# IDSIA/hhmarl_2D

Hardware: AMD Instinct MI355X
Metric: env-steps/sec (2v2) (higher is better)
Workload: dtype f64

## Files before the change

### hhmarl_2d_amd/csrc/hh_device.h

```cpp
#ifndef HH_DEVICE_H
#define HH_DEVICE_H

#include <hip/hip_runtime.h>
#include <stdint.h>

#include "hh_abi.h"
#include "hh_envelope.h"
#include "hh_geodesic.h"
#include "hh_math.h"
#include "hh_rng.h"
#include "hh_spec.h"

#ifdef HH_NO_RARE
#define HH_RARE(x) (x)
#define HH_USUAL(x) (x)
#else
#define HH_RARE(x) __builtin_expect(!!(x), 0)
#define HH_USUAL(x) __builtin_expect(!!(x), 1)
#endif

#ifndef HH_BLOCK
#define HH_BLOCK 64
#endif

// ... 204 lines not shown
    P.cmd_hdg[u] = m.cmd_hdg; P.cmd_spd[u] = m.cmd_spd;
    int4 p;
    p.x = (m.cannon_remain & 0xffff) | ((m.cannon_max & 0xffff) << 16);
    p.y = (m.burst & 0xff) | ((m.missile_remain & 0xff) << 8) | ((m.rocket_max & 0xff) << 16) | ((m.missile_wait & 0xff) << 24);
    p.z = (m.ac_type & 0xff) | ((m.alive & 0xff) << 8) | ((m.has_missile & 0xff) << 16) | ((m.n_tgt & 0xff) << 24);
    p.w = (m.tgt0 & 0xff) | ((m.tgt1 & 0xff) << 8) | ((m.tgt2 & 0xff) << 16) | ((m.cmd_act & 0xff) << 24);
    P.pack[u] = p;
    P.tgt_d[u] = m.tgt_d0; P.tgt_d[U + u] = m.tgt_d1; P.tgt_d[2 * U + u] = m.tgt_d2;
    int2 r;
    r.x = (m.rk_alive & 0xff) | ((m.rk_target & 0xff) << 8) | ((m.rk_life & 0xff) << 16);
    if constexpr (X) {
        const UnitW &x = static_cast<const UnitW &>(m);
        r.x |= (int)(((unsigned)(x.tgt3 & 15) << 24) | ((unsigned)(x.tgt4 & 15) << 28));
        P.tgt_d[3 * U + u] = x.tgt_d3; P.tgt_d[4 * U + u] = x.tgt_d4;
    }
    r.y = m.rk_seq;
    P.rk_pack[u] = r;
    P.rk_lat[u] = m.rk_lat; P.rk_lon[u] = m.rk_lon; P.rk_hdg[u] = m.rk_hdg; P.rk_cmd[u] = m.rk_cmd;
}

__device__ __forceinline__ void arena_load(const DevPtrs &P, const DevCfg &c, int n, Arena &a) {
    int4 p = P.ar_pack[n];
    a.steps = p.x; a.episode = p.y;
    a.escaping = p.z & 0xff; a.escaping_time = (int)(int8_t)((p.z >> 8) & 0xff); a.done = (p.z >> 16) & 0xff;
    a.hl_s = (p.z >> 24) & 0x1f; a.hl_run = (p.z >> 29) & 1;
    a.next_seq = p.w;
    a.akey = hh_rng_arena_key(c.seed, c.arena_offset + (uint64_t)n);
    arena_rekey(a);
}

__device__ __forceinline__ void arena_store(const DevPtrs &P, int n, const Arena &a) {
    int4 p;
    p.x = a.steps; p.y = a.episode;
    p.z = (a.escaping & 0xff) | ((a.escaping_time & 0xff) << 8) | ((a.done & 0xff) << 16) | ((a.hl_s & 0x1f) << 24) | ((a.hl_run & 1) << 29);
    p.w = a.next_seq;
    P.ar_pack[n] = p;
}

__device__ __forceinline__ double d_normalize_angle(double a) {
    while (a >= 360.0) a -= 360.0;
    while (a < 0.0) a += 360.0;
    return a;
}
__device__ __forceinline__ double d_signed_heading_diff(double actual, double desired) {
    double delta = desired - actual;
    if (delta < -180.0) delta = 360.0 + delta;
    if (delta > 180.0) delta = -360.0 + delta;
    return delta;
}

__device__ __forceinline__ void d_dist_bearing(double lat1, double lon1, double lat2, double lon2, double &km, double &brg) {
    double s12, azi1;
    hh_geo_inverse(lat1, lon1, lat2, lon2, &s12, &azi1);
    km = s12 / 1000.0;
    brg = d_normalize_angle(azi1);
}

__device__ __forceinline__ int d_envelope_exact_body(int kind, int ac_type, double la1, double lo1, double la2, double lo2, double hdg) {
    double km, brg;
    d_dist_bearing(la1, lo1, la2, lo2, km, brg);
    if (kind == 0) {
        if (km <= HH_MISSILE_RANGE_KM) {
            double delta = hh_fabs(d_signed_heading_diff(d_normalize_angle(hdg + HH_MISSILE_HALF_DEG), brg));
            return (int)delta <= (int)HH_MISSILE_HALF_DEG;
        }
        return 0;
    }
    if (kind == 1) {
        if (km < HH_AC_CANNON_KM(ac_type)) return hh_fabs(d_signed_heading_diff(hdg, brg)) <= HH_AC_CANNON_HALF(ac_type);
        return 0;
    }
    return km < HH_ROCKET_FUSE_KM;
}
__device__ __noinline__ int d_envelope_exact(int kind, int ac_type, double la1, double lo1, double la2, double lo2, double hdg) {
    return d_envelope_exact_body(kind, ac_type, la1, lo1, la2, lo2, hdg);
}

__device__ __forceinline__ bool d_maybe_within_km(double lat1, double lon1, double lat2, double lon2, double r_km) {
    double lim = r_km / 100.0;
    bool near = hh_fabs(lat2 - lat1) <= lim && hh_fabs(lon2 - lon1) <= lim;
    bool lowlat = hh_fabs(lat1) < 25.0 && hh_fabs(lat2) < 25.0;
    return near || !lowlat;
}

__device__ __noinline__ void d_geo_direct_general(double lat1, double lon1, double azi1, double s12, double *lat2, double *lon2) {
    hh_geo_direct(lat1, lon1, azi1, s12, lat2, lon2);
}
__device__ __forceinline__ void d_geo_move(double lat1, double lon1, double azi1, double s12, double &lat2, double &lon2) {
    double a, b;
    if (HH_USUAL(s12 <= HH_GEO_SHORT_MAX_M && hh_fabs(lat1) <= HH_GEO_SHORT_MAX_LAT && hh_fabs(lon1) < 170.0 && hh_fabs(azi1) <= 360.0))
        hh_geo_direct_short(lat1, lon1, azi1, s12, &a, &b);
    else
        d_geo_direct_general(lat1, lon1, azi1, s12, &a, &b);
    lat2 = a;
    lon2 = b;
}

__device__ __forceinline__ void d_geo_move2(double lat_a, double lon_a, double azi_a, double s_a, double &lat2_a, double &lon2_a,
                                            double lat_b, double lon_b, double azi_b, double s_b, double &lat2_b, double &lon2_b) {
    bool ok_a = s_a <= HH_GEO_SHORT_MAX_M && hh_fabs(lat_a) <= HH_GEO_SHORT_MAX_LAT && hh_fabs(lon_a) < 170.0 && hh_fabs(azi_a) <= 360.0;
    bool ok_b = s_b <= HH_GEO_SHORT_MAX_M && hh_fabs(lat_b) <= HH_GEO_SHORT_MAX_LAT && hh_fabs(lon_b) < 170.0 && hh_fabs(azi_b) <= 360.0;
    if (HH_USUAL(ok_a && ok_b)) {
        double a0, a1, b0, b1;
        hh_geo_direct_short(lat_a, lon_a, azi_a, s_a, &a0, &a1);
        hh_geo_direct_short(lat_b, lon_b, azi_b, s_b, &b0, &b1);
        lat2_a = a0; lon2_a = a1; lat2_b = b0; lon2_b = b1;
    } else {
        d_geo_move(lat_a, lon_a, azi_a, s_a, lat2_a, lon2_a);
        d_geo_move(lat_b, lon_b, azi_b, s_b, lat2_b, lon2_b);
    }
}

__device__ __forceinline__ double d_rng(const Arena &a, int unit_id, int site, int sub) {
    return hh_rng_u01(a.tkey, (uint32_t)unit_id, (uint32_t)site, (uint32_t)sub);
}

#endif
```

### hhmarl_2d_amd/csrc/hh_kernels.h

```cpp
#ifndef HH_KERNELS_H
#define HH_KERNELS_H

#include "hh_device.h"

#ifdef HH_PROFILE_PHASES
__device__ unsigned long long hh_prof_cycles[24];
#define HH_PROF_DECL unsigned long long prof_t0_ = __builtin_readcyclecounter(), prof_acc_[14] = {0}
#define HH_PROF(k) do { unsigned long long t_ = __builtin_readcyclecounter(); prof_acc_[k] += t_ - prof_t0_; prof_t0_ = t_; } while (0)
#define HH_PROF_ARGS , unsigned long long &prof_t0_, unsigned long long *prof_acc_
#define HH_PROF_PASS , prof_t0_, prof_acc_
#define HH_PROF_FLUSH do { if ((threadIdx.x & 63) == 0) { for (int k_ = 0; k_ < 12; k_++) atomicAdd(&hh_prof_cycles[k_], prof_acc_[k_]); \
                                                          atomicAdd(&hh_prof_cycles[20], prof_acc_[12]); atomicAdd(&hh_prof_cycles[21], prof_acc_[13]); } } while (0)
#else
#define HH_PROF_DECL
#define HH_PROF(k)
#define HH_PROF_ARGS
#define HH_PROF_PASS
#define HH_PROF_FLUSH
#endif

template <int A, int B>
struct Shared {
    static constexpr int GPB = B / A;
    double lat0[B], lon0[B], hdg[B];
// ... 236 lines not shown
    if (mode != 2) out[n++] = (sh.flags[o] & FL_SHOT) ? 1.0f : 0.0f;
    return n;
}

template <int A, int B>
__device__ __forceinline__ void friend_block(const DevCfg &c, const Shared<A, B> &sh, int tid, int base, int s, int fj, float *out) {
    const int f = base + fj;
    if (sh_alive(sh, f)) {
        out[0] = sh.nlat[f];
        out[1] = sh.nlon[f];
        out[2] = (float)norm180(sh.p_foc[fj][tid]);
        out[3] = (float)norm180(sh.p_foc[s][f]);
        out[4] = (float)(c.inv_diag * sh.p_dist[fj][tid]);
    } else {
        out[0] = out[1] = out[2] = out[3] = out[4] = 0.0f;
    }
}

template <int A, int B>
__device__ __forceinline__ void lowlevel_obs(const DevCfg &c, const Shared<A, B> &sh, int tid, int base, int s, int mode, Unit &m, float *out, int D) {
    for (int k = 0; k < D; k++) out[k] = 0.0f;
    m.n_tgt = 0; m.tgt0 = 0; m.tgt_d0 = 0.0;
    if (!m.alive) return;
    Near3 nb;
    nearby(c, sh, tid, base, s, false, nb);
    if (nb.n == 0) return;
    m.n_tgt = 1; m.tgt0 = nb.i0 + 1; m.tgt_d0 = nb.d0;
    int fri = s < c.nA ? (s == 1 ? 0 : 1) : (s == 3 ? 2 : 3);
    int n = 0;
    out[n++] = sh.nlat[tid];
    out[n++] = sh.nlon[tid];
    out[n++] = sh.nspd[tid];
    out[n++] = sh.nhdg[tid];
    if (mode == HH_MODE_FIGHT) {
        const int oj = nb.i0;
        out[n++] = (float)norm180(sh.p_foc[oj][tid]);
        out[n++] = (float)aspect(sh.p_foc[s][base + oj]);
        out[n++] = sh.p_hd[oj][tid];
        out[n++] = (float)nb.d0;
        out[n++] = (float)hh_clip((double)m.cannon_remain / (double)m.cannon_max, 0.0, 1.0);
        if (m.ac_type == 1) {
            out[n++] = (float)hh_clip((double)m.missile_remain / (double)m.rocket_max, 0.0, 1.0);
            out[n++] = m.missile_wait == 0 ? 1.0f : 0.0f;
            out[n++] = (m.has_missile || m.burst > 0) ? 1.0f : 0.0f;
        } else {
            out[n++] = m.burst > 0 ? 1.0f : 0.0f;
        }
        n += opp_block(c, sh, 0, tid, base, s, oj, nb.d0, out + n);
    } else {
        out[n++] = (float)hh_clip((double)m.cannon_remain / (double)m.cannon_max, 0.0, 1.0);
        if (m.ac_type == 1) out[n++] = (float)hh_clip((double)m.missile_remain / (double)m.rocket_max, 0.0, 1.0);
        out[n++] = (sh.flags[tid] & FL_SHOT) ? 1.0f : 0.0f;
        opp_block(c, sh, 1, tid, base, s, nb.i0, nb.d0, out + n);
        if (nb.n >= 2) opp_block(c, sh, 1, tid, base, s, nb.i1, nb.d1, out + n + 9);
        n += 18;
    }
    friend_block(c, sh, tid, base, s, fri, out + n);
}

struct StepOut {
    double reward;
    int valid;
    int kill_event;
    double opp_stat0;
};

template <int GS, int B, bool INLINE_EXACT, class SH>
__device__ __forceinline__ void drain_envelope_queue_t(SH &sh, int tid, int count, int opp_id0) {
#ifdef HH_ABL_NO_ENVELOPE
    count = 0;
#endif
#pragma unroll 1
    for (int q = tid; q < count; q += B) {
        int code = sh.u.t.q_code[q];
        int src = code & 0xff, kind = (code >> 8) & 3, j = (code >> 10) & (GS > 8 ? 15 : 7);
        int ss = src % GS, sb = src - ss;
        double la1, lo1, la2, lo2;
        if (kind <= 1) { la1 = sh.lat0[src]; lo1 = sh.lon0[src]; }
        else { la1 = sh.u.t.rk_lat[src]; lo1 = sh.u.t.rk_lon[src]; }
        bool moved = kind >= 2 || (kind == 1 && j < ss);
        la2 = moved ? sh.u.t.lat1[sb + j] : sh.lat0[sb + j];
        lo2 = moved ? sh.u.t.lon1[sb + j] : sh.lon0[sb + j];
        const int t = (sh.flags[src] >> 1) & 3;
        const double hdg_src = kind == 0 ? sh.hdg[src] : sh.u.t.hdg1[src];
        const double sep = hh_max(hh_fabs(la2 - la1), hh_fabs(lo2 - lo1));
        const bool dom = hh_fabs(la1) <= HH_GEO_EST_MAX_LAT && hh_fabs(la2) <= HH_GEO_EST_MAX_LAT &&
                         hh_fabs(lo1) < 170.0 && hh_fabs(lo2) < 170.0;
        int verdict = -1;
        if (dom && sep <= (kind == 0 ? HH_GEO_EST_LONG_DEG : HH_GEO_EST_SHORT_DEG)) {
            double s_m, az;
            hh_geo_inverse_estimate(la1, lo1, la2, lo2, &s_m, &az);
            if (kind == 0) {
                double delta = hh_fabs(d_signed_heading_diff(d_normalize_angle(hdg_src + HH_MISSILE_HALF_DEG), az));
                if (s_m >= HH_MISSILE_RANGE_KM * 1000.0 + HH_GEO_EST_LONG_ABS_M) verdict = 0;
                else if (s_m <= HH_MISSILE_RANGE_KM * 1000.0 - HH_GEO_EST_LONG_ABS_M && s_m > HH_GEO_EST_MIN_M &&
                         hh_fabs(delta - (HH_MISSILE_HALF_DEG + 1.0)) > HH_GEO_EST_LONG_AZI)
                    verdict = delta < HH_MISSILE_HALF_DEG + 1.0;
            } else {
                const double r_m = (kind == 1 ? HH_AC_CANNON_KM(t) : HH_ROCKET_FUSE_KM) * 1000.0;
                const double eps = HH_GEO_EST_SHORT_REL * s_m + HH_GEO_EST_SHORT_ABS_M;
                if (s_m >= r_m + eps) verdict = 0;
                else if (s_m < r_m - eps && s_m > HH_GEO_EST_MIN_M) {
                    if (kind >= 2) verdict = 1;
                    else {
                        double d = hh_fabs(d_signed_heading_diff(hdg_src, az));
                        if (d <= HH_AC_CANNON_HALF(t) - HH_GEO_EST_SHORT_AZI) verdict = 1;
                        else if (d > HH_AC_CANNON_HALF(t) + HH_GEO_EST_SHORT_AZI) verdict = 0;
                    }
                }
            }
        }
#ifndef HH_ABL_NO_EXACT
        if (HH_RARE(verdict < 0)) verdict = INLINE_EXACT ? d_envelope_exact_body(kind, t, la1, lo1, la2, lo2, hdg_src)
                                                : d_envelope_exact(kind, t, la1, lo1, la2, lo2, hdg_src);
#endif
        int bit = 0;
        if (verdict) {
            if (kind == 0) bit = 1;
            else if (kind == 1) {
                const int id_src = GS == 8 ? (ss < 4 ? ss + 1 : opp_id0 + (ss - 4)) : ss + 1;
                const int id_tgt = GS == 8 ? (j < 4 ? j + 1 : opp_id0 + (j - 4)) : j + 1;
                double u = hh_rng_u01(sh.g_tkey[src / GS], (uint32_t)id_src, HH_SITE_CANNON, (uint32_t)id_tgt);
                if (u < HH_AC_HIT_PROB(t)) bit = 2 << j;
            } else bit = kind == 2 ? (1 << HH_RES_FUSE_BIT(GS)) : (1 << (HH_RES_FUSE_BIT(GS) + 1));
        }
        if (bit) atomicOr(&sh.res[src], bit);
    }
}
template <int A, int B, bool INLINE_EXACT = false>
__device__ __forceinline__ void drain_envelope_queue(Shared<A, B> &sh, int tid, int count) {
    drain_envelope_queue_t<A, B, INLINE_EXACT>(sh, tid, count, 0);
}

__device__ __forceinline__ void arm_cannon(Unit &m) {
    int b = HH_AC_BURST(m.ac_type);
    m.burst = m.cannon_remain < b ? m.cannon_remain : b;
}

template <int A, int B>
__device__ __forceinline__ int launch_planar(const Shared<A, B> &sh, int tid, int base, int j) {
    const double la = sh.lat0[tid], lo = sh.lon0[tid], tl = sh.lat0[base + j], to = sh.lon0[base + j];
    const double cross = sh.uc[tid] * (tl - la) - sh.us[tid] * (to - lo);
    return hh_missile_cone_planar(la, lo, tl, to, sh.p_foc[j][tid], cross, sh.p_dist[j][tid]);
}

template <int A, int B>
__device__ __forceinline__ int launch_planar_direct(const Shared<A, B> &sh, int tid, int base, int j) {
    const double la = sh.lat0[tid], lo = sh.lon0[tid], tl = sh.lat0[base + j], to = sh.lon0[base + j];
    const double c1 = sh.uc[tid], s1 = sh.us[tid], n1 = sh.un[tid];
    const double dx = to - lo, dy = tl - la;
    const double n2 = hh_sqrt(dx * dx + dy * dy);
    const double x = hh_clip((c1 * dx + s1 * dy) / (n1 * n2 + 1e-10), -1.0, 1.0);
    return hh_missile_cone_planar(la, lo, tl, to, hh_acos(x) * (180.0 / HH_PI), c1 * dy - s1 * dx, n2);
}

template <int A, int B, bool IX = false>
__device__ __forceinline__ void tick(const DevCfg &c, Shared<A, B> &sh, int tid, int g, int s, int base, bool active,
                                     Unit &m, Arena &ar, const int8_t *act, StepOut &out, uint32_t &ev_mask_out,
                                     const int tmode, const bool run_arena HH_PROF_ARGS) {
    const int id = s + 1;
    const bool running = tmode == 0 ? (active && !ar.done) : (active && run_arena);
    const bool agent = s < c.nA;
    const bool hl = c.env_kind == HH_ENV_HIGHLEVEL;
    if (tmode == 0) { out.reward = 0.0; out.valid = 0; }
    uint32_t evm = 0;
    out.kill_event = 0;
    if (running && tmode == 0) { ar.steps += 1; arena_rekey(ar); }
    const bool snap = running && m.alive;
    double opp_stat0 = tmode == 0 ? 0.0 : out.opp_stat0;
    int want_launch = 0, launch_tgt = 0;
    int wait_after = -1;
    bool base_gate = false;

    if (snap && tmode == 0) {
        if (agent || c.ext_opp) {
            int t = m.n_tgt ? m.tgt0 : 0;
            if (!agent) {
                Near3 nb;
                nearby(c, sh, tid, base, s, false, nb);
                m.n_tgt = nb.n ? 1 : 0; m.tgt0 = nb.n ? nb.i0 + 1 : 0; m.tgt_d0 = nb.n ? nb.d0 : 0.0;
                t = m.tgt0;
            } else {
                out.valid = 1;
                if (t && sh_alive(sh, base + t - 1)) opp_stat0 = norm180(sh.p_foc[s][base + t - 1]);
            }
            double nh = hh_pymod360(m.hdg + (double)(((int)act[0] - 6) * 15));
            if (nh >= 360.0 || nh < 0.0) nh = 0.0;
            m.cmd_hdg = nh;
            double mx = HH_AC_MAX_SPEED(m.ac_type);
            m.cmd_spd = 100.0 + ((mx - 100.0) / 8.0) * (double)act[1];
            bool agent_ll = agent && !hl;
            if (act[2] && m.cannon_remain > 0) {
                arm_cannon(m);
                if (agent_ll && c.agent_mode == HH_MODE_ESCAPE && m.cannon_remain < 90) out.reward -= 0.1;
            }
            if (m.ac_type == 1 && act[3]) {
                if (t && m.missile_remain > 0 && !m.has_missile && m.missile_wait == 0) {
                    base_gate = true;
                    want_launch = 1;
                    launch_tgt = t - 1;
                }
            }
        } else if (c.level <= 2) {
            if (c.level == 2) {
                arm_cannon(m);
                bool man = ar.steps <= 5;
                if (!man) man = (ar.steps % hh_rng_randint(d_rng(ar, id, HH_SITE_L2_PERIOD, 0), 35, 45)) <= 5;
// ... 739 lines not shown
```

### hhmarl_2d_amd/csrc/hh_kernels_oct.h

```cpp
#ifndef HH_KERNELS_OCT_H
#define HH_KERNELS_OCT_H

#include "hh_kernels_hier.h"

#define HH_DPP_QP(a, b, c, d) ((a) | ((b) << 2) | ((c) << 4) | ((d) << 6))
#define HH_DPP_ROW_SHL(n) (0x100 + (n))
#define HH_DPP_ROW_SHR(n) (0x110 + (n))

template <int CTRL>
__device__ __forceinline__ int o_perm_i(int v) { return __builtin_amdgcn_mov_dpp(v, CTRL, 0xf, 0xf, true); }
__device__ __forceinline__ int o_swap_i(int v) {
    const int a = __builtin_amdgcn_update_dpp(v, v, HH_DPP_ROW_SHL(4), 0xf, 0x5, false);
    return __builtin_amdgcn_update_dpp(a, v, HH_DPP_ROW_SHR(4), 0xf, 0xa, false);
}
template <int K>
__device__ __forceinline__ int o_rot_i(int v) {
    static_assert(K == 1 || K == 2, "ring of three");
    return o_perm_i<(K == 1 ? HH_DPP_QP(1, 2, 0, 3) : HH_DPP_QP(2, 0, 1, 3))>(v);
}
template <int P>
__device__ __forceinline__ int o_bc_i(int v) {
    const int t = o_perm_i<HH_DPP_QP(P & 3, P & 3, P & 3, P & 3)>(v);
    if (P < 4) return __builtin_amdgcn_update_dpp(t, t, HH_DPP_ROW_SHR(4), 0xf, 0xa, false);
    return __builtin_amdgcn_update_dpp(t, t, HH_DPP_ROW_SHL(4), 0xf, 0x5, false);
// ... 388 lines not shown
    out.kill_event = 0;
    const bool snap = running && L.exists && m.alive;
    const int amask0 = tb.amask;
    const int rk_age0 = (m.rk_alive && m.rk_life <= HH_ROCKET_MAX_LIFE) ? m.rk_life : 0;
    const double rk_speed0 = sh.rk_speed[rk_age0];

    const double lat_old = m.lat, lon_old = m.lon, hdg_old = m.hdg;
    bool fired = false;
    const int rk_pre = m.rk_alive;
    if (HH_USUAL(snap)) {
        const int t = m.ac_type;
        {
            const double delta = d_signed_heading_diff(m.hdg, m.cmd_hdg);
            const double max_deg = HH_AC_TURN_RATE(t) * 1.0;
            const double stepped = hh_pymod360(m.hdg + (delta >= 0.0 ? max_deg : -max_deg));
            const double nh = hh_fabs(delta) <= max_deg ? m.cmd_hdg : stepped;
            m.hdg = m.hdg != m.cmd_hdg ? nh : m.hdg;
        }
        {
            const double delta = m.cmd_spd - m.spd;
            const double max_delta = HH_AC_ACCEL(t) * 1.0;
            const double stepped = m.spd + (delta >= 0.0 ? max_delta : -max_delta);
            const double ns = hh_fabs(delta) <= max_delta ? m.cmd_spd : stepped;
            m.spd = m.spd != m.cmd_spd ? ns : m.spd;
        }
        {
            const bool f = m.burst > 0;
            const int b1 = m.burst - 1 > 0 ? m.burst - 1 : 0, c1 = m.cannon_remain - 1 > 0 ? m.cannon_remain - 1 : 0;
            fired = f;
            m.burst = f ? b1 : m.burst;
            m.cannon_remain = f ? c1 : m.cannon_remain;
        }
    }
    {
        const bool steer = snap & (m.has_missile != 0) & (m.rk_alive != 0);
        if (HH_USUAL(steer)) m.rk_cmd = hh_clip(m.rk_hdg * hh_rng_uniform(d_rng(ar, id, HH_SITE_ROCKET_NOISE, 0), 0.95, 1.05), 0.0, 359.0);
        m.has_missile = (snap & (m.has_missile != 0) & (m.rk_alive == 0)) ? 0 : m.has_missile;
    }
    const bool rk_spec = running && L.exists && rk_pre && m.rk_life <= HH_ROCKET_MAX_LIFE;
    double rk_nlat = 0.0, rk_nlon = 0.0, rk_nhdg = 0.0;
    {
        const bool mv_a = snap && m.spd > 0.0;
        const bool any_rk = __ballot(rk_spec) != 0ULL;
        if (HH_USUAL(any_rk)) {
            double r_hdg = m.rk_hdg;
            const double r_cmd = m.rk_cmd;
            {
                const double delta = d_signed_heading_diff(r_hdg, r_cmd);
                const double stepped = r_hdg + (delta >= 0.0 ? HH_ROCKET_TURN_RATE : -HH_ROCKET_TURN_RATE);
                const double nh = hh_fabs(delta) <= HH_ROCKET_TURN_RATE ? r_cmd : stepped;
                r_hdg = r_hdg != r_cmd ? nh : r_hdg;
            }
            rk_nhdg = r_hdg;
            double a_lat, a_lon;
            d_geo_move2(m.lat, m.lon, m.hdg, mv_a ? m.spd * HH_KNOTS_TO_MS * 1.0 : 0.0, a_lat, a_lon,
                        rk_spec ? m.rk_lat : 5.0, rk_spec ? m.rk_lon : 7.0, r_hdg, rk_speed0 * HH_KNOTS_TO_MS * 1.0, rk_nlat, rk_nlon);
            if (mv_a) { m.lat = a_lat; m.lon = a_lon; }
        } else {
            if (mv_a) d_geo_move(m.lat, m.lon, m.hdg, m.spd * HH_KNOTS_TO_MS * 1.0, m.lat, m.lon);
        }
    }
    const double rk0_lat = rk_pre ? m.rk_lat : lat_old, rk0_lon = rk_pre ? m.rk_lon : lon_old;
    OPub pn = pub;
    oct_publish_vec(m, pn);
    if (FULL) oct_publish_norm(c, m, pn);
    double lat1[5], lon1[5];
    HH_O_FETCH5(d, lat1, m.lat);
    HH_O_FETCH5(d, lon1, m.lon);

    const bool rk_maybe = running && L.exists && rk_pre;
    int q_total = 0;
    {
        const int t = m.ac_type;
        int push[5], pjs[5], any_push = 0;
#pragma unroll
        for (int r = 0; r < 5; r++) {
            const int pj = o_rel_pos(L, r);
            const bool snap_j = running && ((amask0 >> pj) & 1);
            const bool enemy = r >= 2;
            const bool lower = pj < L.p;
            const double tl = lower ? lat1[r] : tb.lat[r];
            const double to = lower ? lon1[r] : tb.lon[r];
            push[r] = (int)fired & (int)snap_j & ((int)(c.friendly_kill != 0) | (int)enemy) & (int)d_maybe_within_km(lat_old, lon_old, tl, to, HH_AC_CANNON_KM(t)) &
                      (int)!hh_cannon_cone_planar_outside(lat_old, lon_old, tl, to, pn.uc, pn.us, t);
            pjs[r] = pj;
            any_push |= push[r];
        }
        if (HH_RARE(o_any(any_push != 0))) {
#pragma unroll
            for (int r = 0; r < 5; r++) HH_O_PUSH(push[r] != 0, tid | (1 << 8) | (pjs[r] << 10));
        }
        if (o_any(rk_maybe)) {
            const int tp = rk_maybe ? o_slot_pos(c, m.rk_target - 1) : ((1 - L.q) << 2);
            const int rt = o_pos_rel(L, tp);
            HH_O_PUSH(rk_maybe && d_maybe_within_km(rk0_lat, rk0_lon, o_sel5(lat1, rt), o_sel5(lon1, rt), HH_ROCKET_FUSE_KM), tid | (2 << 8) | (tp << 10));
            const int fp = o_slot_pos(c, s == 1 ? 0 : 1);
            const bool self = fp == L.p;
            const int rf = self ? 0 : o_pos_rel(L, fp);
            const double fl_ = self ? m.lat : o_sel5(lat1, rf), fo_ = self ? m.lon : o_sel5(lon1, rf);
            HH_O_PUSH(rk_maybe && c.friendly_kill && d_maybe_within_km(rk0_lat, rk0_lon, fl_, fo_, HH_ROCKET_FUSE_KM), tid | (3 << 8) | (fp << 10));
        }
    }
    int myres = 0;
    if (HH_RARE(q_total != 0)) {
        sh.lat0[tid] = lat_old; sh.lon0[tid] = lon_old; sh.hdg[tid] = hdg_old;
        sh.flags[tid] = pub.flags;
        sh.u.t.lat1[tid] = m.lat; sh.u.t.lon1[tid] = m.lon; sh.u.t.hdg1[tid] = m.hdg;
        sh.u.t.rk_lat[tid] = rk0_lat; sh.u.t.rk_lon[tid] = rk0_lon;
        sh.res[tid] = 0;
        if (L.p == 0) sh.g_tkey[L.g] = ar.tkey;
        o_wave_sync();
        drain_envelope_queue_t<8, 64, IX>(sh, tid, q_total, c.nA + 1);
        o_wave_sync();
        myres = sh.res[tid];
    }
    const int rk_at_start = m.rk_alive;
    const int aux = fired ? (myres >> 1) & 0xff : 0;
    int rkw = 0;
    if (HH_USUAL(running && L.exists && rk_at_start)) {
        const int eol = m.rk_life > HH_ROCKET_MAX_LIFE;
        rkw = 1 | (((myres >> 9) & 1) << 1) | (((myres >> 10) & 1) << 2) | (eol << 3) | (o_slot_pos(c, m.rk_target - 1) << 4) | (m.rk_seq << 8);
    }

    int alive = amask0, nev = 0, dead = 0;
    unsigned long long evpack = 0;
    if (HH_RARE(__ballot(aux != 0 || (rkw & 0xe) != 0) != 0ULL)) {
        int aux_[8], res_[8];
        aux_[0] = o_bc_i<0>(aux); aux_[1] = o_bc_i<1>(aux); aux_[2] = o_bc_i<2>(aux);
        aux_[4] = o_bc_i<4>(aux); aux_[5] = o_bc_i<5>(aux); aux_[6] = o_bc_i<6>(aux);
        res_[0] = o_bc_i<0>(rkw); res_[1] = o_bc_i<1>(rkw); res_[2] = o_bc_i<2>(rkw);
        res_[4] = o_bc_i<4>(rkw); res_[5] = o_bc_i<5>(rkw); res_[6] = o_bc_i<6>(rkw);
        aux_[3] = aux_[7] = res_[3] = res_[7] = 0;
        if (running) {
            if (aux_[0] | aux_[1] | aux_[2] | aux_[4] | aux_[5] | aux_[6]) {
#pragma unroll
                for (int i = 0; i < 7; i++) {
                    if (i == 3) continue;
                    const int ci = aux_[i];
#pragma unroll
                    for (int j = 0; j < 7; j++) {
                        if (j == 3) continue;
                        if (((ci >> j) & 1) && ((alive >> j) & 1)) {
                            alive &= ~(1 << j);
                            evpack |= (unsigned long long)(i | (j << 3)) << (7 * nev);
                            nev++;
                        }
                    }
                }
            }
            int done_mask = 0;
#pragma unroll 1
            for (int k = 0; k < 6; k++) {
                int best = -1, best_seq = 0x7fffffff, w = 0;
#pragma unroll
                for (int j = 0; j < 7; j++) {
                    if (j == 3) continue;
                    const int wj = res_[j];
                    if ((wj & 1) && !((done_mask >> j) & 1) && (wj >> 8) < best_seq) { best = j; best_seq = wj >> 8; w = wj; }
                }
                if (best < 0) break;
                done_mask |= 1 << best;
                const int tg = (w >> 4) & 7;
                const int fid = o_slot_pos(c, o_pos_slot(c, best) == 1 ? 0 : 1);
                if (((w >> 1) & 1) && ((alive >> tg) & 1)) {
                    alive &= ~(1 << tg); dead |= 1 << best;
                    evpack |= (unsigned long long)(best | (tg << 3) | (1 << 6)) << (7 * nev);
                    nev++;
// ... 650 lines not shown
```

### include/hh_envelope.h

```cpp
#ifndef HH_ENVELOPE_H
#define HH_ENVELOPE_H

#include "hh_geodesic.h"
#include "hh_spec.h"

#define HH_PLANAR_MIN_DEG 0.01
#define HH_PLANAR_AZI_MARGIN 0.5
HH_HD int hh_missile_cone_planar(double lat1, double lon1, double lat2, double lon2, double focus_deg, double cross,
                                 double sep_deg) {
    const int dom = (hh_fabs(lat1) <= HH_GEO_EST_MAX_LAT) & (hh_fabs(lat2) <= HH_GEO_EST_MAX_LAT) & (hh_fabs(lon1) < 170.0) &
                    (hh_fabs(lon2) < 170.0) & (sep_deg >= HH_PLANAR_MIN_DEG) & (sep_deg <= HH_GEO_EST_LONG_DEG);
    const double beta = cross < 0.0 ? focus_deg : -focus_deg;
    const int inside = (beta >= -1.0 + HH_PLANAR_AZI_MARGIN) & (beta <= (HH_MISSILE_HALF_DEG * 2.0 + 1.0) - HH_PLANAR_AZI_MARGIN);
    const int outside = (beta < -1.0 - HH_PLANAR_AZI_MARGIN) | (beta > (HH_MISSILE_HALF_DEG * 2.0 + 1.0) + HH_PLANAR_AZI_MARGIN);
    const int r = inside ? 1 : (outside ? 0 : -1);
    return dom ? r : -1;
}

#define HH_PLANAR_CONE_MARGIN 0.3
#define HH_COS_5P3_DEG 0.9957246981845821
#define HH_COS_3P8_DEG 0.99780146829205
HH_HD int hh_cannon_cone_planar_outside(double lat1, double lon1, double lat2, double lon2, double he, double hn, int ac_type) {
    const double dx = lon2 - lon1, dy = lat2 - lat1;
    const int dom = (hh_fabs(lat1) <= HH_GEO_EST_MAX_LAT) & (hh_fabs(lat2) <= HH_GEO_EST_MAX_LAT) & (hh_fabs(lon1) < 170.0) &
                    (hh_fabs(lon2) < 170.0) & (hh_fabs(dx) <= HH_GEO_EST_SHORT_DEG) & (hh_fabs(dy) <= HH_GEO_EST_SHORT_DEG);
    const double d2 = dx * dx + dy * dy;
    const int ok = dom & !(d2 < 1e-10);
    const double dot = he * dx + hn * dy;
    const double h2 = he * he + hn * hn;
    const double cw = ac_type == 1 ? HH_COS_5P3_DEG : HH_COS_3P8_DEG;
    return ok & ((dot <= 0.0) | (dot * dot < (cw * cw) * (d2 * h2)));
}

#endif
```

### include/hh_geodesic.h

```cpp
#ifndef HH_GEODESIC_H
#define HH_GEODESIC_H

#include "hh_math.h"

#define HH_GEO_A 6378137.0
#define HH_GEO_F 0.0033528106647474805
#define HH_GEO_F1 0.9966471893352525
#define HH_GEO_E2 0.0066943799901413165
#define HH_GEO_EP2 0.006739496742276434
#define HH_GEO_N 0.0016792203863837047
#define HH_GEO_B 6356752.314245179
#define HH_GEO_ETOL2 3.6424611488788524e-08
#define HH_GEO_TINY 1.4916681462400413e-154
#define HH_GEO_TOL0 2.220446049250313e-16
#define HH_GEO_MAXIT 20

HH_HD double hh_geo_clenshaw6(double sinx, double cosx, const double *c) {
    double ar = 2.0 * (cosx - sinx) * (cosx + sinx);
    double y0 = 0.0, y1 = 0.0;
    y1 = ar * y0 - y1 + c[6];
    y0 = ar * y1 - y0 + c[5];
    y1 = ar * y0 - y1 + c[4];
    y0 = ar * y1 - y0 + c[3];
    y1 = ar * y0 - y1 + c[2];
// ... 166 lines not shown

typedef struct { double S0, C0, U0, W0, iC, hW; } hh_geo_lat_terms;
HH_HD hh_geo_lat_terms hh_geo_short_lat_terms(double lat1) {
    hh_geo_lat_terms t;
    hh_sincosd_small(lat1, &t.S0, &t.C0);
    t.U0 = hh_fma(-HH_GEO_E2 * t.S0, t.S0, 1.0);
    t.W0 = hh_sqrt(t.U0);
    t.iC = 1.0 / t.C0;
    t.hW = 0.5 / t.W0;
    return t;
}
HH_HD void hh_geo_direct_short_core(double lat1, double lon1, double azi1, double s12, hh_geo_lat_terms lt, double *lat2, double *lon2) {
    const double E2 = HH_GEO_E2, K1 = 1.0 / (1.0 - HH_GEO_E2), TH = 1.0 / 3.0, M2E2 = -2.0 * HH_GEO_E2;
    const double S0 = lt.S0, C0 = lt.C0, U0 = lt.U0, W0 = lt.W0, iC = lt.iC, hW = lt.hW;
    double Sa0, Ca0;
    hh_sincosd_small(azi1, &Sa0, &Ca0);
    const double h = s12 * (1.0 / HH_GEO_A);
    const double Q0 = W0 * iC, P0 = W0 * U0 * K1;
    const double f1 = Ca0 * P0;
    const double SS0 = Sa0 * S0;
    const double a1 = SS0 * Q0;
    const double l1 = Sa0 * Q0;
    const double S1 = C0 * f1, C1 = -S0 * f1, Sa1 = Ca0 * a1, Ca1 = -Sa0 * a1;
    const double U1 = (M2E2 * S0) * S1;
    const double W1 = U1 * hW;
    const double Q1 = hh_fma(-C1, Q0, W1) * iC;
    const double P1 = hh_fma(W0, U1, W1 * U0) * K1;
    const double g2 = hh_fma(Ca0, P1, Ca1 * P0);
    const double f2 = 0.5 * g2;
    const double SS1 = hh_fma(Sa0, S1, Sa1 * S0);
    const double h2 = hh_fma(SS0, Q1, SS1 * Q0);
    const double l2 = 0.5 * hh_fma(Sa0, Q1, Sa1 * Q0);
    const double S2 = 0.5 * hh_fma(C0, g2, C1 * f1), C2 = -0.5 * hh_fma(S0, g2, S1 * f1);
    const double Sa2 = 0.5 * hh_fma(Ca0, h2, Ca1 * a1), Ca2 = -0.5 * hh_fma(Sa0, h2, Sa1 * a1);
    const double U2 = -E2 * hh_fma(2.0 * S0, S2, S1 * S1);
    const double W2 = hh_fma(-W1, W1, U2) * hW;
    const double Q2 = hh_fma(-C2, Q0, hh_fma(-C1, Q1, W2)) * iC;
    const double P2 = hh_fma(W0, U2, hh_fma(W1, U1, W2 * U0)) * K1;
    const double g3 = hh_fma(Ca0, P2, hh_fma(Ca1, P1, Ca2 * P0));
    const double f3 = TH * g3;
    const double l3 = TH * hh_fma(Sa0, Q2, hh_fma(Sa1, Q1, Sa2 * Q0));
    const double dphi = h * hh_fma(h, hh_fma(h, f3, f2), f1);
    const double dlam = h * hh_fma(h, hh_fma(h, l3, l2), l1);
    *lat2 = hh_fma(dphi, HH_RAD2DEG, lat1);
    *lon2 = hh_fma(dlam, HH_RAD2DEG, lon1);
}
HH_HD void hh_geo_direct_short(double lat1, double lon1, double azi1, double s12, double *lat2, double *lon2) {
    hh_geo_direct_short_core(lat1, lon1, azi1, s12, hh_geo_short_lat_terms(lat1), lat2, lon2);
}

HH_HD void hh_geo_move(double lat1, double lon1, double azi1, double s12, double *lat2, double *lon2) {
    if (s12 <= HH_GEO_SHORT_MAX_M && hh_fabs(lat1) <= HH_GEO_SHORT_MAX_LAT && hh_fabs(lon1) < 170.0 && hh_fabs(azi1) <= 360.0)
        hh_geo_direct_short(lat1, lon1, azi1, s12, lat2, lon2);
    else
        hh_geo_direct(lat1, lon1, azi1, s12, lat2, lon2);
}


#define HH_GEO_EST_MAX_LAT 10.0
#define HH_GEO_EST_SHORT_DEG 0.06
#define HH_GEO_EST_LONG_DEG 0.85
#define HH_GEO_EST_SHORT_REL 1e-6
#define HH_GEO_EST_SHORT_ABS_M 1e-3
#define HH_GEO_EST_SHORT_AZI 1e-4
#define HH_GEO_EST_LONG_ABS_M 10.0
#define HH_GEO_EST_LONG_AZI 1e-2
#define HH_GEO_EST_MIN_M 1.0

HH_HD void hh_geo_inverse_estimate(double lat1, double lon1, double lat2, double lon2, double *s12, double *azi1) {
    double pm = (0.5 * (lat1 + lat2)) * HH_DEG2RAD;
    double dp = (lat2 - lat1) * HH_DEG2RAD, dl = (lon2 - lon1) * HH_DEG2RAD;
    double sm, cm;
    hh_sincos(pm, &sm, &cm);
    double W2 = 1.0 - HH_GEO_E2 * sm * sm;
    double W = hh_sqrt(W2);
    double N = HH_GEO_A / W;
    double M = N * (1.0 - HH_GEO_E2) / W2;
    double x = N * cm * dl, y = M * dp;
    *s12 = hh_sqrt(x * x + y * y);
    double a = (hh_atan2(x, y) - 0.5 * dl * sm) * HH_RAD2DEG;
    if (a < 0.0) a += 360.0;
    if (a >= 360.0) a -= 360.0;
    *azi1 = a;
}

HH_HD void hh_geo_lengths(double eps, double sig12, double ssig1, double csig1, double dn1, double ssig2,
                          double csig2, double dn2, double *s12b, double *m12b) {
    double C1a[7], C2a[7];
    double A1 = hh_geo_A1m1f(eps);
    hh_geo_C1f(eps, C1a);
    double A2 = hh_geo_A2m1f(eps);
    hh_geo_C2f(eps, C2a);
    double m0x = A1 - A2;
    A2 = 1.0 + A2;
    A1 = 1.0 + A1;
    double B1 = hh_geo_clenshaw6(ssig2, csig2, C1a) - hh_geo_clenshaw6(ssig1, csig1, C1a);
    *s12b = A1 * (sig12 + B1);
    double B2 = hh_geo_clenshaw6(ssig2, csig2, C2a) - hh_geo_clenshaw6(ssig1, csig1, C2a);
    double J12 = m0x * sig12 + (A1 * B1 - A2 * B2);
    *m12b = dn2 * (csig1 * ssig2) - dn1 * (ssig1 * csig2) - csig1 * csig2 * J12;
}

typedef struct {
    double lam12, salp2, calp2, sig12, ssig1, csig1, ssig2, csig2, eps, dlam12;
} hh_geo_l12;

HH_HD void hh_geo_lambda12(double sbet1, double cbet1, double dn1, double sbet2, double cbet2, double dn2,
                           double salp1, double calp1, double slam120, double clam120, hh_geo_l12 *o) {
    double C3a[6];
    if (sbet1 == 0.0 && calp1 == 0.0) calp1 = -HH_GEO_TINY;
    double salp0 = salp1 * cbet1;
    double calp0 = hh_hypot(calp1, salp1 * sbet1);
    double ssig1 = sbet1, somg1 = salp0 * sbet1;
    double csig1 = calp1 * cbet1, comg1 = csig1;
    hh_geo_norm(&ssig1, &csig1);
    double salp2 = cbet2 != cbet1 ? salp0 / cbet2 : salp1;
    double calp2;
    if (cbet2 != cbet1 || hh_fabs(sbet2) != -sbet1) {
        double t = cbet1 < -sbet1 ? (cbet2 - cbet1) * (cbet1 + cbet2) : (sbet1 - sbet2) * (sbet1 + sbet2);
        double cc = calp1 * cbet1;
        calp2 = hh_sqrt(cc * cc + t) / cbet2;
    } else {
        calp2 = hh_fabs(calp1);
    }
    double ssig2 = sbet2, somg2 = salp0 * sbet2;
    double csig2 = calp2 * cbet2, comg2 = csig2;
    hh_geo_norm(&ssig2, &csig2);
    double sig12 = hh_atan2(hh_max(0.0, csig1 * ssig2 - ssig1 * csig2) + 0.0, csig1 * csig2 + ssig1 * ssig2);
    double somg12 = hh_max(0.0, comg1 * somg2 - somg1 * comg2) + 0.0;
    double comg12 = comg1 * comg2 + somg1 * somg2;
    double eta = hh_atan2(somg12 * clam120 - comg12 * slam120, comg12 * clam120 + somg12 * slam120);
    double k2 = calp0 * calp0 * HH_GEO_EP2;
    double eps = k2 / (2.0 * (1.0 + hh_sqrt(1.0 + k2)) + k2);
    hh_geo_C3f(eps, C3a);
    double B312 = hh_geo_clenshaw5(ssig2, csig2, C3a) - hh_geo_clenshaw5(ssig1, csig1, C3a);
    double domg12 = -HH_GEO_F * hh_geo_A3f(eps) * salp0 * (sig12 + B312);
    o->lam12 = eta + domg12;
    if (calp2 == 0.0) {
        o->dlam12 = -2.0 * HH_GEO_F1 * dn1 / sbet1;
    } else {
        double s12b, m12b;
        hh_geo_lengths(eps, sig12, ssig1, csig1, dn1, ssig2, csig2, dn2, &s12b, &m12b);
        o->dlam12 = m12b * HH_GEO_F1 / (calp2 * cbet2);
    }
    o->salp2 = salp2; o->calp2 = calp2; o->sig12 = sig12;
    o->ssig1 = ssig1; o->csig1 = csig1; o->ssig2 = ssig2; o->csig2 = csig2; o->eps = eps;
}

HH_HD void hh_geo_inverse(double lat1, double lon1, double lat2, double lon2, double *s12_out, double *azi1_out) {
    double lon12s;
    double lon12 = hh_ang_diff(lon1, lon2, &lon12s);
    double lonsign = hh_copysign(1.0, lon12);
    lon12 = lonsign * lon12;
    lon12s = lonsign * lon12s;
    double lam12 = lon12 * HH_DEG2RAD;
    double slam12, clam12;
    hh_sincosde(lon12, lon12s, &slam12, &clam12);
    lon12s = (180.0 - lon12) - lon12s;
    lat1 = hh_ang_round(lat1);
    lat2 = hh_ang_round(lat2);
    double swapp = hh_fabs(lat1) < hh_fabs(lat2) ? -1.0 : 1.0;
    if (swapp < 0.0) {
        lonsign = -lonsign;
        double t = lat1; lat1 = lat2; lat2 = t;
    }
    double latsign = hh_copysign(1.0, -lat1);
// ... 112 lines not shown
```

Baseline: 966.1 million.

## Draw cannon hit RNG before geometry and skip envelope work on misses

In the envelope drain loop, the cannon hit random draw now runs before the geodesic check, and queue entries whose draw misses skip the geometry test entirely. Rocket fuse entries use a range-only inverse estimate that leaves out the atan2 azimuth. The oct kernel's cannon-cone prefilter drops the short-separation domain limit, so more pairs are decided by the planar test without exact geometry. This cuts transcendental and exact-geodesic work, at the cost of an RNG draw for every cannon entry and possible wave divergence from the early continue.

```diff
diff --git a/hhmarl_2d_amd/csrc/hh_device.h b/hhmarl_2d_amd/csrc/hh_device.h
--- a/hhmarl_2d_amd/csrc/hh_device.h
+++ b/hhmarl_2d_amd/csrc/hh_device.h
@@ -310,6 +310,11 @@
     bool lowlat = hh_fabs(lat1) < 25.0 && hh_fabs(lat2) < 25.0;
     return near || !lowlat;
 }
+#ifdef HH_ABL_CONE_DOMAIN
+#define HH_CANNON_CONE_OUTSIDE_NEAR hh_cannon_cone_planar_outside
+#else
+#define HH_CANNON_CONE_OUTSIDE_NEAR hh_cannon_cone_planar_outside_near
+#endif
 
 __device__ __noinline__ void d_geo_direct_general(double lat1, double lon1, double azi1, double s12, double *lat2, double *lon2) {
     hh_geo_direct(lat1, lon1, azi1, s12, lat2, lon2);
diff --git a/hhmarl_2d_amd/csrc/hh_kernels.h b/hhmarl_2d_amd/csrc/hh_kernels.h
--- a/hhmarl_2d_amd/csrc/hh_kernels.h
+++ b/hhmarl_2d_amd/csrc/hh_kernels.h
@@ -342,13 +342,31 @@
         la2 = moved ? sh.u.t.lat1[sb + j] : sh.lat0[sb + j];
         lo2 = moved ? sh.u.t.lon1[sb + j] : sh.lon0[sb + j];
         const int t = (sh.flags[src] >> 1) & 3;
+#ifndef HH_ABL_DRAW_LAST
+        int hit_bit = 0;
+        if (kind == 1) {
+            const int id_src = GS == 8 ? (ss < 4 ? ss + 1 : opp_id0 + (ss - 4)) : ss + 1;
+            const int id_tgt = GS == 8 ? (j < 4 ? j + 1 : opp_id0 + (j - 4)) : j + 1;
+            const double u = hh_rng_u01(sh.g_tkey[src / GS], (uint32_t)id_src, HH_SITE_CANNON, (uint32_t)id_tgt);
+            hit_bit = u < HH_AC_HIT_PROB(t) ? (2 << j) : 0;
+        }
+        const bool geometry = kind != 1 || hit_bit != 0;
+#ifdef HH_PROFILE_PHASES
+        if (__ballot(geometry) == 0ULL && q == tid && tid == 0) atomicAdd(&hh_prof_cycles[22], 1ULL);
+#endif
+        if (!geometry) continue;
+#endif
         const double hdg_src = kind == 0 ? sh.hdg[src] : sh.u.t.hdg1[src];
         const double sep = hh_max(hh_fabs(la2 - la1), hh_fabs(lo2 - lo1));
         const bool dom = hh_fabs(la1) <= HH_GEO_EST_MAX_LAT && hh_fabs(la2) <= HH_GEO_EST_MAX_LAT &&
                          hh_fabs(lo1) < 170.0 && hh_fabs(lo2) < 170.0;
         int verdict = -1;
         if (dom && sep <= (kind == 0 ? HH_GEO_EST_LONG_DEG : HH_GEO_EST_SHORT_DEG)) {
-            double s_m, az;
+            double s_m, az = 0.0;
+#ifndef HH_ABL_DRAW_LAST
+            if (kind >= 2) hh_geo_inverse_estimate_range(la1, lo1, la2, lo2, &s_m);
+            else
+#endif
             hh_geo_inverse_estimate(la1, lo1, la2, lo2, &s_m, &az);
             if (kind == 0) {
                 double delta = hh_fabs(d_signed_heading_diff(d_normalize_angle(hdg_src + HH_MISSILE_HALF_DEG), az));
@@ -377,12 +395,17 @@
         int bit = 0;
         if (verdict) {
             if (kind == 0) bit = 1;
+#ifndef HH_ABL_DRAW_LAST
+            else if (kind == 1) bit = hit_bit;
+#else
             else if (kind == 1) {
                 const int id_src = GS == 8 ? (ss < 4 ? ss + 1 : opp_id0 + (ss - 4)) : ss + 1;
                 const int id_tgt = GS == 8 ? (j < 4 ? j + 1 : opp_id0 + (j - 4)) : j + 1;
                 double u = hh_rng_u01(sh.g_tkey[src / GS], (uint32_t)id_src, HH_SITE_CANNON, (uint32_t)id_tgt);
                 if (u < HH_AC_HIT_PROB(t)) bit = 2 << j;
-            } else bit = kind == 2 ? (1 << HH_RES_FUSE_BIT(GS)) : (1 << (HH_RES_FUSE_BIT(GS) + 1));
+            }
+#endif
+            else bit = kind == 2 ? (1 << HH_RES_FUSE_BIT(GS)) : (1 << (HH_RES_FUSE_BIT(GS) + 1));
         }
         if (bit) atomicOr(&sh.res[src], bit);
     }
diff --git a/hhmarl_2d_amd/csrc/hh_kernels_oct.h b/hhmarl_2d_amd/csrc/hh_kernels_oct.h
--- a/hhmarl_2d_amd/csrc/hh_kernels_oct.h
+++ b/hhmarl_2d_amd/csrc/hh_kernels_oct.h
@@ -494,7 +494,7 @@
             const double tl = lower ? lat1[r] : tb.lat[r];
             const double to = lower ? lon1[r] : tb.lon[r];
             push[r] = (int)fired & (int)snap_j & ((int)(c.friendly_kill != 0) | (int)enemy) & (int)d_maybe_within_km(lat_old, lon_old, tl, to, HH_AC_CANNON_KM(t)) &
-                      (int)!hh_cannon_cone_planar_outside(lat_old, lon_old, tl, to, pn.uc, pn.us, t);
+                      (int)!HH_CANNON_CONE_OUTSIDE_NEAR(lat_old, lon_old, tl, to, pn.uc, pn.us, t);
             pjs[r] = pj;
             any_push |= push[r];
         }
diff --git a/include/hh_envelope.h b/include/hh_envelope.h
--- a/include/hh_envelope.h
+++ b/include/hh_envelope.h
@@ -32,4 +32,15 @@
     return ok & ((dot <= 0.0) | (dot * dot < (cw * cw) * (d2 * h2)));
 }
 
+HH_HD int hh_cannon_cone_planar_outside_near(double lat1, double lon1, double lat2, double lon2, double he, double hn, int ac_type) {
+    const double dx = lon2 - lon1, dy = lat2 - lat1;
+    const int dom = (hh_fabs(lat1) <= HH_GEO_EST_MAX_LAT) & (hh_fabs(lat2) <= HH_GEO_EST_MAX_LAT) & (hh_fabs(lon1) < 170.0) & (hh_fabs(lon2) < 170.0);
+    const double d2 = dx * dx + dy * dy;
+    const int ok = dom & !(d2 < 1e-10);
+    const double dot = he * dx + hn * dy;
+    const double h2 = he * he + hn * hn;
+    const double cw = ac_type == 1 ? HH_COS_5P3_DEG : HH_COS_3P8_DEG;
+    return ok & ((dot <= 0.0) | (dot * dot < (cw * cw) * (d2 * h2)));
+}
+
 #endif
diff --git a/include/hh_geodesic.h b/include/hh_geodesic.h
--- a/include/hh_geodesic.h
+++ b/include/hh_geodesic.h
@@ -272,6 +272,18 @@
     if (a < 0.0) a += 360.0;
     if (a >= 360.0) a -= 360.0;
     *azi1 = a;
+}
+HH_HD void hh_geo_inverse_estimate_range(double lat1, double lon1, double lat2, double lon2, double *s12) {
+    double pm = (0.5 * (lat1 + lat2)) * HH_DEG2RAD;
+    double dp = (lat2 - lat1) * HH_DEG2RAD, dl = (lon2 - lon1) * HH_DEG2RAD;
+    double sm, cm;
+    hh_sincos(pm, &sm, &cm);
+    double W2 = 1.0 - HH_GEO_E2 * sm * sm;
+    double W = hh_sqrt(W2);
+    double N = HH_GEO_A / W;
+    double M = N * (1.0 - HH_GEO_E2) / W2;
+    double x = N * cm * dl, y = M * dp;
+    *s12 = hh_sqrt(x * x + y * y);
 }
 
 HH_HD void hh_geo_lengths(double eps, double sig12, double ssig1, double csig1, double dn1, double ssig2,
```

Measured after the change: 992.8 million, median of 6. 2.8% higher.
